# i4Ds/whisper-finetune

Measured on AMD Instinct MI355X. Metric: audio-seconds/sec training throughput, whisper-large-v3 bf16, higher is better.
Workload: dtype bf16; 1 GPU; whisper-large-v3 full fine-tune, AdamW, bf16 MFMA / fp32 master weights, 96 synthetic 30 s clips per GPU per step, decoder S=128, log-mel + SpecAugment on GPU, label smoothing 0.1, clip 1.0, local accumulation 1 (global window = 1); timed loop = model_utils.train_step; global_batch=96, seq_len=128, parallelism=dp1

## Files before the change

### include/wft.h

```cpp
#ifndef WFT_H
#define WFT_H

#include <stdint.h>

#ifdef __cplusplus
extern "C" {
#endif

typedef enum {
  WFT_OK = 0,
  WFT_ERR_ARG = -1,
  WFT_ERR_LAUNCH = -2,
  WFT_ERR_UNSUPPORTED = -3
} wft_status;

typedef uint16_t wft_bf16;

const char* wft_last_error(void);
const char* wft_version(void);

int wft_cast_f32_bf16(const float* src, wft_bf16* dst, int64_t n, void* stream);
int wft_cast_bf16_f32(const wft_bf16* src, float* dst, int64_t n, void* stream);
int wft_cast_pad_transpose_f32_bf16(const float* src, int64_t rows, int64_t cols,
                                    wft_bf16* dst, wft_bf16* dst_t,
// ... 75 lines not shown
} wft_gemm_args;
int wft_gemm_nt_bf16(const wft_gemm_args* args, void* stream);
int wft_gemm_nt_variant(const wft_gemm_args* args);
int wft_gemm_tn_segments_ok(const wft_gemm_args* args);
int64_t wft_gemm_nt_colsum_workspace_bytes(const wft_gemm_args* args);
int64_t wft_gemm_nt_splitk_workspace_bytes(const wft_gemm_args* args);
int64_t wft_gemm_nt_aux8_bytes(const wft_gemm_args* args);
int wft_gemm_nt_stream_bf16(const wft_gemm_args* args, void* stream);
int wft_gemm_nt_stream_ok(const wft_gemm_args* args);
int64_t wft_gemm_nt_stream_workspace_bytes(const wft_gemm_args* args);
int wft_gemm_nt_stream_q8(const wft_gemm_args* args, const float* b_scale, void* stream);
int wft_gemm_nt_stream_q8_ok(const wft_gemm_args* args);
int64_t wft_gemm_nt_stream_q8_workspace_bytes(const wft_gemm_args* args);
int wft_gemm_tn_bf16(const wft_gemm_args* args, void* stream);
int wft_gemm_tn_variant(const wft_gemm_args* args);
int wft_gemm_nt_rank_pair_bf16(const wft_gemm_args* args0, const wft_gemm_args* args1, void* stream);
int wft_gemm_tn_rank_pair_bf16(const wft_gemm_args* args0, const wft_gemm_args* args1, void* stream);
int64_t wft_gemm_tn_workspace_bytes(const wft_gemm_args* args);

typedef struct {
  const wft_bf16* q; int64_t ldq; int64_t q_bs;
  const wft_bf16* k; int64_t ldk; int64_t k_bs;
  const wft_bf16* v; int64_t ldv; int64_t v_bs;
  wft_bf16* o; int64_t ldo; int64_t o_bs;
  float* lse;
  int B; int H; int Tq; int Tk; int causal; float scale;
  const wft_bf16* d_o; int64_t lddo; int64_t do_bs;
  float* delta;
  wft_bf16* dq; int64_t lddq; int64_t dq_bs;
  wft_bf16* dk; int64_t lddk; int64_t dk_bs;
// ... 177 lines not shown
```

### whisper-finetune_amd/csrc/gemm.hip

```cpp
#include "gemm_common.h"
#include <stdlib.h>

struct TnReduceP {
  const float* ws; float* C; long ldc; int P, Q, nsplit, accumulate, Pz; const float* col_scale; int scale_rows, blk_n, blk_r, Pv;
};
__device__ __forceinline__ void tn_splitk_reduce_body(const float* ws, float* C, long ldc, int P, int Q, int nsplit,
                                                      int accumulate, int Pz, const float* col_scale, int scale_rows,
                                                      int blk_n, int blk_r, int Pv, long bid, long nblk) {
  const long nq4 = Q >> 2;
  const long total = (long)(Pz > P ? Pz : P) * nq4;
  for (long i = bid * 256 + threadIdx.x; i < total; i += nblk * 256) {
    const long pp = i / nq4, q4 = (i - pp * nq4) * 4;
    float* cp = C + pp * ldc + q4;
    if (col_scale && blk_n == 0 && pp >= Pv) continue;
    if (pp >= P) {
      if (!accumulate && blk_n == 0) *(f32x4*)cp = f32x4{0.f, 0.f, 0.f, 0.f};
      continue;
    }
    int pr = 0;
    float* ob = nullptr;
    if (blk_n > 0) {
      const int blk = (int)(q4 / blk_n);
      pr = (int)pp - blk * blk_r;
      if (pr < 0 || pr >= blk_r) continue;
      ob = C + (long)blk * blk_n * blk_r + (q4 - (long)blk * blk_n) * blk_r + pr;
    }
    const bool plain = !col_scale && !ob;
    f32x4 s = (plain && accumulate) ? *(const f32x4*)cp : f32x4{0.f, 0.f, 0.f, 0.f};
    for (int k = 0; k < nsplit; ++k) s += *(const f32x4*)(ws + ((long)k * P + pp) * Q + q4);
    if (plain) {
      *(f32x4*)cp = s;
      continue;
    }
    if (col_scale && pp < Pv) s *= *(const f32x4*)(col_scale + (scale_rows > 0 ? pp / scale_rows : 0) * Q + q4);
    if (ob) {
#pragma unroll
      for (int e = 0; e < 4; ++e) ob[(long)e * blk_r] = accumulate ? ob[(long)e * blk_r] + s[e] : s[e];
    } else {
      if (accumulate) s += *(const f32x4*)cp;
      *(f32x4*)cp = s;
    }
  }
}

__global__ __launch_bounds__(256) void tn_splitk_reduce_kernel(const float* ws, float* C, long ldc, int P, int Q, int nsplit,
                                                                int accumulate, int Pz, const float* col_scale, int scale_rows,
                                                                int blk_n, int blk_r, int Pv) {
  tn_splitk_reduce_body(ws, C, ldc, P, Q, nsplit, accumulate, Pz, col_scale, scale_rows, blk_n, blk_r, Pv, (long)blockIdx.x, (long)gridDim.x);
}
struct TnSegs { float* ptr[4]; int end[4]; };
__global__ __launch_bounds__(256) void tn_splitk_reduce_seg_kernel(const float* ws, TnSegs sg, int P, int Q, int nsplit, int accumulate) {
  const long nq4 = Q >> 2;
  const long total = (long)P * nq4;
  for (long i = (long)blockIdx.x * 256 + threadIdx.x; i < total; i += (long)gridDim.x * 256) {
    const long pp = i / nq4, q4 = (i - pp * nq4) * 4;
    int sgi = 0, start = 0;
    while (sgi < 3 && pp >= sg.end[sgi]) start = sg.end[sgi++];
    float* cp = sg.ptr[sgi] + (pp - start) * Q + q4;
    f32x4 s = accumulate ? *(const f32x4*)cp : f32x4{0.f, 0.f, 0.f, 0.f};
    for (int k = 0; k < nsplit; ++k) s += *(const f32x4*)(ws + ((long)k * P + pp) * Q + q4);
    *(f32x4*)cp = s;
  }
}
__global__ __launch_bounds__(256) void tn_splitk_reduce_pair_kernel(TnReduceP r0, TnReduceP r1, int g0) {
  const bool second = (int)blockIdx.x >= g0;
  const TnReduceP& r = second ? r1 : r0;
  tn_splitk_reduce_body(r.ws, r.C, r.ldc, r.P, r.Q, r.nsplit, r.accumulate, r.Pz, r.col_scale, r.scale_rows, r.blk_n, r.blk_r, r.Pv,
                        (long)blockIdx.x - (second ? g0 : 0), (long)(second ? (int)gridDim.x - g0 : g0));
}

static const int g_diag = [] { const char* e = wft_dev_getenv("WFT_GEMM_DIAG"); return e ? atoi(e) : 0; }();
static const int g_nt256_band = [] { const char* e = wft_dev_getenv("WFT_NT256_BAND"); return (e && atoi(e) > 0) ? atoi(e) : 5; }();

static void fill_params(const wft_gemm_args* a, GemmP& p) {
  p.A = a->A; p.lda = a->lda; p.sA = a->strideA;
  p.B = a->B; p.ldb = a->ldb; p.sB = a->strideB;
  p.C = a->C; p.ldc = a->ldc; p.sC = a->strideC;
  p.bias = a->bias;
  p.res = a->residual; p.ldr = a->ldr; p.sR = a->strideR;
  p.aux = a->aux; p.ldaux = a->ldaux; p.sAux = a->strideAux;
  p.alpha = a->alpha;
  p.beta = a->beta == 0.f ? 1.f : a->beta;
  p.M = (int)a->M; p.N = (int)a->N; p.K = (int)a->K; p.batch = a->batch;
  p.accumulate = a->accumulate;
  p.period = a->valid_rows_period; p.valid = a->valid_rows;
  p.res_first = a->residual_first;
  p.diag = g_diag;
  p.band = g_nt256_band;
  p.ws = nullptr;
  p.cs_part = nullptr;
  p.nsplit = 1;
}

static bool ws_granted(const wft_gemm_args* a, int64_t bytes) {
  return a->workspace && a->workspace_bytes >= bytes && (((uintptr_t)a->workspace) & 15) == 0;
}

static int gemm_check_common(const wft_gemm_args* a, const char* who) {
  WFT_CHECK_ARG_AS(who, a->lda % 8 == 0 && a->ldb % 8 == 0 && a->ldc % 4 == 0, "ld alignment");
  WFT_CHECK_ARG_AS(who, ((uintptr_t)a->A & 15) == 0 && ((uintptr_t)a->B & 15) == 0 && ((uintptr_t)a->C & 15) == 0,
                   "base pointers must be 16-byte aligned");
  WFT_CHECK_ARG_AS(who, !(a->accumulate && !a->c_is_f32), "accumulate needs an f32 C");
  return WFT_OK;
}

static const int g_force_128 = [] { const char* e = wft_dev_getenv("WFT_GEMM_FORCE_128"); return (e && e[0] == '1') ? 1 : 0; }();
// ... 108 lines not shown
}

static bool tn_uses_256(const wft_gemm_args* a) {
  const long nsteps = ((a->K + 63) / 64) * a->batch;
  const long t256 = (a->M / 256) * (a->N / 256);
  return !g_force_128 && a->c_is_f32 && a->M % 256 == 0 && a->N % 256 == 0 && nsteps >= g_tn256_min_steps &&
         (nsteps >= 256 || t256 >= g_tn256_min_out_tiles || (t256 >= g_tn256_min_out_tiles / 2 && nsteps >= 128));
}
static bool tn_needs_reduce(const wft_gemm_args* a) { return a->tn_col_scale != nullptr || a->tn_block_n > 0; }
static const int g_tn_variant = [] { const char* e = wft_dev_getenv("WFT_TN_VARIANT"); return (e && e[0] == 'p') ? 1 : 0; }();

struct TnPlan {
  TnKind kind = TN_128_2BUF;
  long tiles = 0;
  int nsplit = 1, per = 0;
  int pb = 0;
  int64_t ws_rows = 0;
  int64_t part_bytes = 0;
  int64_t ws_bytes = 0;
  bool use_ws = false;
};
static TnPlan tn_plan(const wft_gemm_args* a) {
  TnPlan pl;
  if (!a) return pl;
  const bool seg = a->tn_seg_count > 0;
  const auto part = [&](int nsplit) { return (int64_t)nsplit * pl.ws_rows * a->N * 4; };
  if (tn_uses_256(a)) {
    pl.tiles = (a->M / 256) * (a->N / 256);
    pl.ws_rows = a->M;
    const int ns256 = wft_tn256_nsplit(a);
    int ns4 = 0, per4 = 0;
    const bool elig4 = wft_tn4w_eligible(a);
    if (elig4) wft_tn4w_plan(a, &ns4, &per4);
    const int nsq = ns4 > ns256 ? ns4 : ns256;
    pl.ws_bytes = (nsq > 1 || seg || tn_needs_reduce(a)) ? part(nsq) : 0;
    if (elig4 && g_tn_variant != 1 && a->variant == 0) {
      const bool use4 = (ns4 > 1 || seg) && ws_granted(a, part(ns4));
      if (ns4 == 1 || use4) {
        pl.kind = TN_4W; pl.nsplit = ns4; pl.per = per4; pl.use_ws = use4; pl.part_bytes = part(ns4);
        return pl;
      }
    }
    pl.kind = TN_256; pl.nsplit = ns256; pl.part_bytes = part(ns256);
    pl.use_ws = (ns256 > 1 || seg) && ws_granted(a, pl.part_bytes);
    return pl;
  }
  pl.tiles = (a->M / 128) * (a->N / 128);
  const bool ring = wft_tn128_ring(a, g_diag);
  pl.nsplit = wft_tn128_nsplit(a, ring);
  pl.pb = wft_tn128_pb(a);
  pl.ws_rows = pl.pb ? 16 * pl.pb : a->M;
  pl.part_bytes = part(pl.nsplit);
  const bool want_ws = pl.nsplit > 1 || tn_needs_reduce(a);
  pl.ws_bytes = (want_ws || seg) ? pl.part_bytes : 0;
  pl.use_ws = want_ws && ws_granted(a, pl.part_bytes);
  if (pl.pb > 0 && (pl.nsplit == 1 || pl.use_ws)) pl.kind = TN_RANK;
  else if (!a->c_is_f32) pl.kind = TN_128_BF16C;
  else if (pl.pb > 0) pl.kind = TN_128_PB;
  else pl.kind = ring ? TN_128_RING : TN_128_2BUF;
  return pl;
}

extern "C" int wft_gemm_tn_segments_ok(const wft_gemm_args* a) {
  const TnKind k = tn_plan(a).kind;
  if ((k != TN_4W && k != TN_256) || a->tn_seg_count < 1 || a->tn_seg_count > 4 || tn_needs_reduce(a) || a->p_valid != 0 || a->batch != 1) return 0;
  int prev = 0;
  for (int i = 0; i < a->tn_seg_count; ++i) {
    if (a->tn_seg_end[i] <= prev || !a->tn_seg_ptr[i] || (((uintptr_t)a->tn_seg_ptr[i]) & 15) != 0) return 0;
    prev = a->tn_seg_end[i];
  }
  return prev == a->M ? 1 : 0;
}
extern "C" int64_t wft_gemm_tn_workspace_bytes(const wft_gemm_args* a) { return tn_plan(a).ws_bytes; }
extern "C" int wft_gemm_tn_variant(const wft_gemm_args* a) {
  const TnKind k = tn_plan(a).kind;
  return k == TN_4W ? 4 : k == TN_256 ? 256 : 128;
}

static int tn_check(const wft_gemm_args* a, const TnPlan& pl, const char* who) {
  WFT_CHECK_ARG_AS(who, a && a->A && a->B && a->C, "null pointer");
  WFT_CHECK_ARG_AS(who, a->M >= 128 && a->N >= 128 && a->K >= 1 && a->batch >= 1, "bad shape");
  WFT_CHECK_ARG_AS(who, a->M % 128 == 0 && a->N % 128 == 0, "P and Q must be multiples of 128");
  const int rc = gemm_check_common(a, who);
  if (rc != WFT_OK) return rc;
  WFT_CHECK_ARG_AS(who, a->M < (1ll << 31) && a->N < (1ll << 31) && a->K < (1ll << 31), "dims exceed int32");
  if (tn_needs_reduce(a)) {
    WFT_CHECK_ARG_AS(who, pl.pb > 0, "tn_col_scale / tn_block_n need a rank-r operand (P = 128, 0 < p_valid <= 64)");
    WFT_CHECK_ARG_AS(who, ws_granted(a, pl.ws_bytes), "tn_col_scale / tn_block_n need the workspace of wft_gemm_tn_workspace_bytes");
    WFT_CHECK_ARG_AS(who, a->tn_scale_rows >= 0 && (((uintptr_t)a->tn_col_scale) & 15) == 0, "tn_col_scale: 16-byte aligned f32 [S][Q]");
    if (a->tn_block_n > 0)
      WFT_CHECK_ARG_AS(who, a->tn_block_n % 4 == 0 && a->N % a->tn_block_n == 0 && a->tn_block_r >= 1 &&
                       (a->N / a->tn_block_n) * (int64_t)a->tn_block_r <= 16 * pl.pb, "tn_block_n / tn_block_r do not tile the product");
  }
// ... 6 lines not shown
static TnSegs tn_segs_of(const wft_gemm_args* a) {
  TnSegs sg;
  for (int i = 0; i < 4; ++i) {
    const int j = i < a->tn_seg_count ? i : a->tn_seg_count - 1;
    sg.ptr[i] = a->tn_seg_ptr[j];
    sg.end[i] = i < a->tn_seg_count ? a->tn_seg_end[i] : 0x7fffffff;
  }
  return sg;
}
static unsigned tn_reduce_grid(const wft_gemm_args* a) {
  const long g = (a->M * (a->N / 4) + 255) / 256;
  return (unsigned)(g > 2048 ? 2048 : g);
}
static TnReduceP tn_reduce_params(const wft_gemm_args* a, const TnPlan& pl) {
  return TnReduceP{(const float*)a->workspace, (float*)a->C, (long)a->ldc, (int)pl.ws_rows, (int)a->N, pl.nsplit, a->accumulate, (int)a->M,
                   a->tn_col_scale, a->tn_scale_rows, a->tn_block_n, a->tn_block_r, pl.pb > 0 ? a->p_valid : (int)a->M};
}
static void launch_tn_reduce(const wft_gemm_args* a, const TnPlan& pl, hipStream_t s) {
  const dim3 grid(tn_reduce_grid(a)), block(256);
  if (a->tn_seg_count > 0) {
    hipLaunchKernelGGL(tn_splitk_reduce_seg_kernel, grid, block, 0, s, (const float*)a->workspace, tn_segs_of(a), (int)a->M, (int)a->N,
                       pl.nsplit, a->accumulate);
    return;
  }
  const TnReduceP r = tn_reduce_params(a, pl);
  hipLaunchKernelGGL(tn_splitk_reduce_kernel, grid, block, 0, s, r.ws, r.C, r.ldc, r.P, r.Q, r.nsplit, r.accumulate, r.Pz, r.col_scale,
                     r.scale_rows, r.blk_n, r.blk_r, r.Pv);
}

extern "C" int wft_gemm_tn_bf16(const wft_gemm_args* a, void* stream) {
  const TnPlan pl = tn_plan(a);
  int rc = tn_check(a, pl, __func__);
  if (rc != WFT_OK) return rc;
  GemmP p;
  fill_params(a, p);
  hipStream_t s = (hipStream_t)stream;
  if (pl.use_ws) p.ws = (float*)a->workspace;
  else if (pl.nsplit > 1 && !a->accumulate)
    (void)hipMemset2DAsync(a->C, (size_t)a->ldc * 4, 0, (size_t)a->N * 4, (size_t)a->M, s);
  const unsigned grid1d = (unsigned)(pl.tiles * pl.nsplit);
  switch (pl.kind) {
    case TN_4W:
      p.nsplit = pl.nsplit;
      p.band = pl.per;
      rc = wft_tn4w_launch(p, grid1d, stream);
      break;
    case TN_256:
      p.nsplit = pl.nsplit;
      rc = wft_tn256_launch(p, grid1d, s);
      break;
    case TN_RANK:
      p.nsplit = pl.nsplit;
      rc = wft_tn_rank_launch(pl.pb, p, p, (int)grid1d, 0, s);
      break;
    default: rc = wft_tn128_launch(p, pl.kind, pl.pb, dim3((unsigned)pl.tiles, (unsigned)pl.nsplit), s); break;
  }
  if (rc != WFT_OK) return rc;
  if (pl.use_ws) launch_tn_reduce(a, pl, s);
  WFT_CHECK_LAUNCH();
// ... 24 lines not shown
  bool paired = pl[0].pb == pl[1].pb;
  for (int i = 0; i < 2 && paired; ++i)
    paired = pl[i].kind == TN_RANK && ws_granted(as[i], pl[i].part_bytes) && tn_check(as[i], pl[i], __func__) == WFT_OK;
  if (!paired) {
    const int rc = wft_gemm_tn_bf16(a0, stream);
    return rc != WFT_OK ? rc : wft_gemm_tn_bf16(a1, stream);
  }
  hipStream_t s = (hipStream_t)stream;
  GemmP p[2];
  TnReduceP r[2];
  int nb[2], gr[2];
  for (int i = 0; i < 2; ++i) {
    fill_params(as[i], p[i]);
    p[i].ws = (float*)as[i]->workspace;
    p[i].nsplit = pl[i].nsplit;
    nb[i] = (int)(pl[i].tiles * pl[i].nsplit);
    gr[i] = (int)tn_reduce_grid(as[i]);
    r[i] = tn_reduce_params(as[i], pl[i]);
  }
  const int rc = wft_tn_rank_launch(pl[0].pb, p[0], p[1], nb[0], nb[1], s);
  if (rc != WFT_OK) return rc;
  hipLaunchKernelGGL(tn_splitk_reduce_pair_kernel, dim3((unsigned)(gr[0] + gr[1])), dim3(256), 0, s, r[0], r[1], gr[0]);
  WFT_CHECK_LAUNCH();
  return WFT_OK;
}
```

### whisper-finetune_amd/csrc/gemm_common.h

```cpp
#pragma once
#include "common.h"
#include <type_traits>

struct GemmP {
  const unsigned short* A; long lda; long sA;
  const unsigned short* B; long ldb; long sB;
  void* C; long ldc; long sC;
  const float* bias;
  const unsigned short* res; long ldr; long sR;
  unsigned short* aux; long ldaux; long sAux;
  float alpha, beta;
  int M, N, K, batch;
  int accumulate;
  int period, valid;
  int res_first;
  float* ws;
  float* cs_part;
  int nsplit;
  int band;
  int diag;
};

__device__ __forceinline__ void band_coords(int sid, int tiles_r, int tiles_c, int& tr, int& tc, int W = 5) {
  const int band = sid / (tiles_r * W);
  const int c0 = band * W;
  const int w = (tiles_c - c0) < W ? (tiles_c - c0) : W;
  const int r = sid - band * tiles_r * W;
  tr = r / w;
  tc = c0 + r - tr * w;
}

__device__ __forceinline__ int xcd_remap(int bid, int ntile) {
  const int q = ntile >> 3, r = ntile & 7, xcd = bid & 7;
  return (xcd < r ? xcd * (q + 1) : r * (q + 1) + (xcd - r) * q) + (bid >> 3);
}

template <int IMM>
__device__ __forceinline__ bf16x8 lds_b128_asm(unsigned lds_byte_addr) {
  bf16x8 r;
  asm volatile("ds_read_b128 %0, %1 offset:%2" : "=v"(r) : "v"(lds_byte_addr), "n"(IMM));
  return r;
}
template <int IMM>
__device__ __forceinline__ s16x4 tn_tr_asm(unsigned lds_byte_addr) {
// ... 53 lines not shown
    case WFT_EPI_NONE: return either(EpiC<WFT_EPI_NONE>{});
    case WFT_EPI_GELU: return either(EpiC<WFT_EPI_GELU>{});
    case WFT_EPI_DGELU: return either(EpiC<WFT_EPI_DGELU>{});
    case WFT_EPI_GELU_GRAD: return f(EpiC<WFT_EPI_GELU_GRAD>{}, std::false_type{});
    case WFT_EPI_MUL_AUX: return f(EpiC<WFT_EPI_MUL_AUX>{}, std::false_type{});
    default: wft_set_error("wft_gemm_nt_bf16: unknown epilogue %d", a->epilogue); return WFT_ERR_ARG;
  }
}

enum NtKind { NT_4W, NT_256, NT_RANK, NT_128_SPLITK, NT_128_RING, NT_128_2BUF };
enum TnKind { TN_4W, TN_256, TN_RANK, TN_128_PB, TN_128_RING, TN_128_2BUF, TN_128_BF16C };
bool wft_nt4w_eligible(const wft_gemm_args* a);
int wft_nt4w_launch(const wft_gemm_args* a, const GemmP& p, unsigned grid, void* stream);
bool wft_tn4w_eligible(const wft_gemm_args* a);
void wft_tn4w_plan(const wft_gemm_args* a, int* nsplit_out, int* per_out);
int wft_tn4w_launch(const GemmP& p, unsigned grid, void* stream);
int wft_nt256_launch(const wft_gemm_args* a, const GemmP& p, unsigned grid, hipStream_t s);
void wft_nt_colsum_reduce_launch(const wft_gemm_args* a, hipStream_t s);
int wft_tn256_nsplit(const wft_gemm_args* a);
int wft_tn256_launch(const GemmP& p, unsigned grid, hipStream_t s);
bool wft_nt128_ring(const wft_gemm_args* a, int diag);
int wft_nt128_splitk_plan(const wft_gemm_args* a, int diag, int* per_out);
int wft_nt128_launch(const wft_gemm_args* a, const GemmP& p, NtKind kind, int nsplit, int per, dim3 grid, hipStream_t s);
bool wft_tn128_ring(const wft_gemm_args* a, int diag);
int wft_tn128_nsplit(const wft_gemm_args* a, bool ring);
int wft_tn128_pb(const wft_gemm_args* a);
int wft_tn128_launch(const GemmP& p, TnKind kind, int pb, dim3 grid, hipStream_t s);
int wft_nt_rank_pb(const wft_gemm_args* a);
int wft_nt_rank_launch(int pb, const GemmP& p0, const GemmP& p1, int n0, int n1, hipStream_t s);
int wft_tn_rank_launch(int pb, const GemmP& p0, const GemmP& p1, int n0, int n1, hipStream_t s);
// ... 1 lines not shown
```

### whisper-finetune_amd/csrc/gemm_tn4w.hip

```cpp
#include "gemm_common.h"
#include <stdlib.h>
#include <type_traits>

#define TN4W_BLK 1056
#define TN4W_OP (32 * TN4W_BLK)
#define TN4W_BUF (2 * TN4W_OP)
#define TN4W_LDS (2 * TN4W_BUF)

#define TN4W_STR2(x) #x
#define TN4W_STR(x) TN4W_STR2(x)

#ifndef TN4W_SPP
#define TN4W_SPP 12
#endif
#ifndef TN4W_SPQ
#define TN4W_SPQ 12
#endif
#define TN4W_ASM_MACROS ".set TN4W_SPP, " TN4W_STR(TN4W_SPP) "\n.set TN4W_SPQ, " TN4W_STR(TN4W_SPQ) "\n" R"ASM(
.macro TN4W_MFMA s, z
  .if \z
    v_mfma_f32_16x16x32_bf16 a[4*((\s)%%64):4*((\s)%%64)+3], v[128+64*((\s)/64)+4*((\s)%%8):128+64*((\s)/64)+4*((\s)%%8)+3], v[160+64*((\s)/64)+4*(((\s)%%64)/8):160+64*((\s)/64)+4*(((\s)%%64)/8)+3], 0
  .else
    v_mfma_f32_16x16x32_bf16 a[4*((\s)%%64):4*((\s)%%64)+3], v[128+64*((\s)/64)+4*((\s)%%8):128+64*((\s)/64)+4*((\s)%%8)+3], v[160+64*((\s)/64)+4*(((\s)%%64)/8):160+64*((\s)/64)+4*(((\s)%%64)/8)+3], a[4*((\s)%%64):4*((\s)%%64)+3]
  .endif
// ... 240 lines not shown
__device__ __forceinline__ unsigned tn4w_sgpr(unsigned x) { return __builtin_amdgcn_readfirstlane(x); }
__device__ __forceinline__ unsigned long long tn4w_sgpr64(unsigned long long x) {
  const unsigned lo = __builtin_amdgcn_readfirstlane((unsigned)x), hi = __builtin_amdgcn_readfirstlane((unsigned)(x >> 32));
  return ((unsigned long long)hi << 32) | lo;
}

__global__ __launch_bounds__(256) void gemm_tn4w_kernel(GemmP p) {
  extern __shared__ __attribute__((aligned(16))) char dsmem[];
  const int tid = threadIdx.x, lane = tid & 63;
  const int wave = __builtin_amdgcn_readfirstlane(tid >> 6);
  const int wp = wave >> 1, wq = wave & 1;
  const int P = p.M, Q = p.N, R = p.K;
  const int tiles_q = Q >> 8, tiles_p = P >> 8;
  const int ntile = tiles_p * tiles_q;
  const int nsplit = p.nsplit;
  const int wsid = xcd_remap(blockIdx.x, ntile * nsplit);
  const int split = wsid / ntile, sid = wsid - split * ntile;
  int tp, tq;
  band_coords(sid, tiles_p, tiles_q, tp, tq);
  const int p0 = tp << 8, q0 = tq << 8;
  const int per = p.band;
  const int kb = split * per;
  const int nk_all = (((R + 63) >> 6) + 1) & ~1;
  const int nk = (kb + per <= nk_all) ? per : nk_all - kb;
  const unsigned lds0 = lds_addr_of(dsmem);
  const unsigned lda2 = tn4w_sgpr((unsigned)p.lda * 2u), ldb2 = tn4w_sgpr((unsigned)p.ldb * 2u);

  const int g = lane >> 4, li = lane & 15;
  const unsigned rd0 = lds0 + (unsigned)((li >> 2) + 4 * (g & 1) + 16 * (g >> 1)) * TN4W_BLK + 8u * (li & 3);
  const unsigned rdP0 = rd0 + wp * 256, rdQ0 = rd0 + TN4W_OP + wq * 256;
  const int h = lane >> 5, cp = lane & 31;
  const int rw = 32 * h + 16 * (wave >> 1) + 4 * (wave & 1);
  const unsigned voP = (unsigned)(rw * (int)p.lda + cp * 8) * 2u, voQ = (unsigned)(rw * (int)p.ldb + cp * 8) * 2u;
  const unsigned long long baseP = tn4w_sgpr64((unsigned long long)(p.A + (long)kb * 64 * p.lda + p0));
  const unsigned long long baseQ = tn4w_sgpr64((unsigned long long)(p.B + (long)kb * 64 * p.ldb + q0));
  const long rem = (long)R - (long)kb * 64;
  const unsigned nrP = tn4w_sgpr((unsigned)(rem * p.lda * 2)), nrQ = tn4w_sgpr((unsigned)(rem * p.ldb * 2));
  tn4w_kloop(rdP0, rdQ0, voP, voQ, baseP, baseQ, nrP, nrQ, lda2, ldb2, tn4w_sgpr(lds0 + wave * 8 * TN4W_BLK),
             tn4w_sgpr((unsigned)(nk - 4) >> 1));

  float* const dst = p.ws ? p.ws + ((long)split * P + p0) * Q + q0 : (float*)p.C + (long)p0 * p.ldc + q0;
  const long ldd = p.ws ? (long)Q : p.ldc;
  const bool acc_c = !p.ws && p.accumulate;
  tn4w_for<0, 8>([&](auto fpc) {
    constexpr int fp = decltype(fpc)::value;
    float* const row = dst + (long)(wp * 128 + 16 * fp + li) * ldd + wq * 128 + 4 * g;
    tn4w_for<0, 8>([&](auto fqc) {
      constexpr int fq = decltype(fqc)::value, i0 = (fp * 8 + fq) * 4;
      f32x4 o = {tn4w_acc<i0>(), tn4w_acc<i0 + 1>(), tn4w_acc<i0 + 2>(), tn4w_acc<i0 + 3>()};
      o *= p.alpha;
      if (acc_c) o += *(const f32x4*)(row + 16 * fq);
      *(f32x4*)(row + 16 * fq) = o;
    });
  });
}

bool wft_tn4w_eligible(const wft_gemm_args* a) {
  return a->c_is_f32 && a->batch == 1 && a->M % 256 == 0 && a->N % 256 == 0 && a->K >= 1024 && a->p_valid == 0 && !a->tn_col_scale &&
         a->tn_block_n == 0 && a->lda >= a->M && a->ldb >= a->N && (a->K + 64) * a->lda * 2 < (1ll << 32) &&
         (a->K + 64) * a->ldb * 2 < (1ll << 32);
}
void wft_tn4w_plan(const wft_gemm_args* a, int* nsplit_out, int* per_out) {
  const long t256 = (a->M / 256) * (a->N / 256);
  const long nk = ((((a->K + 63) / 64) + 1) / 2) * 2;
  const int ncu = wft_num_cus();
  int nsplit = 1;
  double best = 0.0;
  for (int sp = 1; sp <= 16; ++sp) {
    if (sp > 1 && nk / sp < 24) break;
    const double waves = (double)(t256 * sp) / (double)ncu;
    const double eff = waves / (double)((long)(waves + 0.999999));
    if (eff > best + 0.02) { best = eff; nsplit = sp; }
  }
  long per = (nk + nsplit - 1) / nsplit;
  per = (per + 1) & ~1l;
  if (per < 4) per = 4;
  long ns = (nk + per - 1) / per;
  while (ns > 1 && nk - (ns - 1) * per < 4) {
    per += 2;
    ns = (nk + per - 1) / per;
  }
  *per_out = (int)per;
  *nsplit_out = (int)ns;
}
int wft_tn4w_launch(const GemmP& p, unsigned grid, void* stream) {
  return wft_launch_lds<gemm_tn4w_kernel>(dim3(grid), dim3(256), TN4W_LDS, (hipStream_t)stream, p);
}
```

### whisper-finetune_amd/whisper_finetune/engine/kernels.py

```python
from __future__ import annotations

import ctypes as C
import math
from typing import Optional

import torch

from . import lib as L

BF16 = torch.bfloat16
F32 = torch.float32

PROFILE_NT = None


def _p(t: Optional[torch.Tensor]):
    return C.c_void_p(0 if t is None else t.data_ptr())


def _chk(t: torch.Tensor, dtype, name: str):
    if t.dtype != dtype:
        raise TypeError(f"{name}: expected {dtype}, got {t.dtype}")
    if not t.is_cuda:
        raise L.WftError(f"{name}: libwft kernels need CUDA/HIP tensors (got {t.device}); there is no CPU path")
# ... 207 lines not shown
            "wft_layernorm_bwd",
        )
    if want_colsum:
        return dx, dgamma, dbeta, dxs
    return dx, dgamma, dbeta


VARIANT = {"nt": 0, "tn": 0, "fwd": 0, "dq": 0, "dkdv": 0}
LAUNCH_OVERRIDE = [None]
LAUNCH_PERSISTENT, LAUNCH_PER_TILE = 0, 1


def set_variant(which: str, v: int) -> int:
    old = VARIANT[which]
    if v >= 0:
        VARIANT[which] = 1 if v else 0
    return old


def _launch(launch: int) -> int:
    o = LAUNCH_OVERRIDE[0]
    return int(launch) if o is None else int(o)


def _attn_variant_bits() -> int:
    return VARIANT["fwd"] | (VARIANT["dq"] << 1) | (VARIANT["dkdv"] << 2)


def gemm_nt(a, b, *, M=None, N=None, K=None, lda=None, ldb=None, out=None, out_f32=False, accumulate=False,
            bias=None, residual=None, aux=None, epilogue=L.EPI_NONE, alpha=1.0, batch=1,
            strideA=0, strideB=0, strideC=0, strideR=0, strideAux=0, ldc=None,
# ... 993 lines not shown
```

### whisper-finetune_amd/whisper_finetune/engine/lib.py

```python
from __future__ import annotations

import ctypes as C
import os
from pathlib import Path

_PKG_ROOT = Path(__file__).resolve().parents[2]
LIB_PATH = Path(os.environ.get("WFT_LIB", _PKG_ROOT / "libwft.so"))

c_i64 = C.c_int64
c_vp = C.c_void_p


class GemmArgs(C.Structure):

    _fields_ = [
        ("A", c_vp), ("lda", c_i64), ("strideA", c_i64),
        ("B", c_vp), ("ldb", c_i64), ("strideB", c_i64),
        ("C", c_vp), ("ldc", c_i64), ("strideC", c_i64), ("c_is_f32", C.c_int), ("accumulate", C.c_int),
        ("bias", c_vp),
        ("residual", c_vp), ("ldr", c_i64), ("strideR", c_i64),
        ("aux", c_vp), ("ldaux", c_i64), ("strideAux", c_i64),
        ("epilogue", C.c_int), ("alpha", C.c_float),
        ("M", c_i64), ("N", c_i64), ("K", c_i64), ("batch", C.c_int),
        ("valid_rows_period", C.c_int), ("valid_rows", C.c_int),
# ... 140 lines not shown
                                C.c_int, c_vp, c_vp],
    "wft_gemm_nt_bf16": [C.POINTER(GemmArgs), c_vp],
    "wft_gemm_nt_variant": [C.POINTER(GemmArgs)],
    "wft_gemm_tn_segments_ok": [C.POINTER(GemmArgs)],
    "wft_gemm_nt_colsum_workspace_bytes": [C.POINTER(GemmArgs)],
    "wft_gemm_nt_splitk_workspace_bytes": [C.POINTER(GemmArgs)],
    "wft_gemm_nt_aux8_bytes": [C.POINTER(GemmArgs)],
    "wft_gemm_nt_stream_bf16": [C.POINTER(GemmArgs), c_vp],
    "wft_gemm_nt_stream_ok": [C.POINTER(GemmArgs)],
    "wft_gemm_nt_stream_workspace_bytes": [C.POINTER(GemmArgs)],
    "wft_gemm_nt_stream_q8": [C.POINTER(GemmArgs), c_vp, c_vp],
    "wft_gemm_nt_stream_q8_ok": [C.POINTER(GemmArgs)],
    "wft_gemm_nt_stream_q8_workspace_bytes": [C.POINTER(GemmArgs)],
    "wft_gemm_tn_bf16": [C.POINTER(GemmArgs), c_vp],
    "wft_gemm_tn_variant": [C.POINTER(GemmArgs)],
    "wft_gemm_nt_rank_pair_bf16": [C.POINTER(GemmArgs), C.POINTER(GemmArgs), c_vp],
    "wft_gemm_tn_rank_pair_bf16": [C.POINTER(GemmArgs), C.POINTER(GemmArgs), c_vp],
    "wft_gemm_tn_workspace_bytes": [C.POINTER(GemmArgs)],
    "wft_attn_fwd_bf16": [C.POINTER(AttnArgs), c_vp],
    "wft_attn_bwd_bf16": [C.POINTER(AttnArgs), c_vp],
    "wft_attn_bwd_colsum_workspace_bytes": [C.POINTER(AttnArgs)],
    "wft_attn_variant": [C.POINTER(AttnArgs), C.c_int],
    "wft_attn_decode_bf16": [C.POINTER(AttnDecodeArgs), c_vp],
    "wft_attn_decode_workspace_bytes": [C.POINTER(AttnDecodeArgs)],
    "wft_decode_embed": [c_vp, c_i64, c_vp, c_vp, c_vp, c_vp, C.c_int, C.c_int, C.c_int, c_i64, c_vp],
    "wft_decode_pick": [C.POINTER(DecodePickArgs), c_vp],
    "wft_attn_decode_beam_bf16": [C.POINTER(AttnDecodeBeamArgs), c_vp],
    "wft_attn_decode_beam_workspace_bytes": [C.POINTER(AttnDecodeBeamArgs)],
    "wft_decode_topk": [C.POINTER(DecodeTopkArgs), c_vp],
    "wft_decode_pick_ts": [C.POINTER(DecodePickArgs), C.POINTER(TsRules), c_vp],
# ... 105 lines not shown
```

Measured before the change: 3620 audio-s/s.

## Add stream-K style balanced split-K scheduling for TN 4-wave weight-gradient GEMM

Adds a balanced work decomposition for the TN 4-wave GEMM. When there are fewer 256x256 tiles than CUs and K is long, each CU gets an equal share of K-steps, and workgroups may walk across tile boundaries into several partial-sum slots. The split-K reduce kernels now work out a per-tile part count so they sum only the slots that were written. This aims to remove wave-quantization tail imbalance in weight-gradient GEMMs. In exchange it adds extra workspace slots, a per-segment fixed cost, and more complex indexing in the kernel and the reduction.

```diff
diff --git a/include/wft.h b/include/wft.h
--- a/include/wft.h
+++ b/include/wft.h
@@ -113,6 +113,10 @@
 int64_t wft_gemm_nt_stream_q8_workspace_bytes(const wft_gemm_args* args);
 int wft_gemm_tn_bf16(const wft_gemm_args* args, void* stream);
 int wft_gemm_tn_variant(const wft_gemm_args* args);
+int wft_gemm_tn_plan(const wft_gemm_args* args, int* out);
+int wft_tn_balanced_segments(int T, int nk, int G, int c, int wg, int* out, int max_segs);
+int wft_tn_balanced_parts(int T, int nk, int G, int c, int tile);
+int wft_tn_balanced_seg_cost(void);
 int wft_gemm_nt_rank_pair_bf16(const wft_gemm_args* args0, const wft_gemm_args* args1, void* stream);
 int wft_gemm_tn_rank_pair_bf16(const wft_gemm_args* args0, const wft_gemm_args* args1, void* stream);
 int64_t wft_gemm_tn_workspace_bytes(const wft_gemm_args* args);
diff --git a/whisper-finetune_amd/csrc/gemm.hip b/whisper-finetune_amd/csrc/gemm.hip
--- a/whisper-finetune_amd/csrc/gemm.hip
+++ b/whisper-finetune_amd/csrc/gemm.hip
@@ -1,12 +1,19 @@
 #include "gemm_common.h"
 #include <stdlib.h>
+#include <algorithm>
 
 struct TnReduceP {
   const float* ws; float* C; long ldc; int P, Q, nsplit, accumulate, Pz; const float* col_scale; int scale_rows, blk_n, blk_r, Pv;
+  int bal_G, bal_nk;
 };
+__device__ __forceinline__ int tn_balanced_parts_at(const TnbPlan& bp, int P, int Q, long pp, long q4) {
+  return tnb_tile_parts(bp, band_index((int)(pp >> 8), (int)(q4 >> 8), P >> 8, Q >> 8));
+}
 __device__ __forceinline__ void tn_splitk_reduce_body(const float* ws, float* C, long ldc, int P, int Q, int nsplit,
                                                       int accumulate, int Pz, const float* col_scale, int scale_rows,
-                                                      int blk_n, int blk_r, int Pv, long bid, long nblk) {
+                                                      int blk_n, int blk_r, int Pv, int bal_G, int bal_nk, long bid, long nblk) {
+  TnbPlan bp;
+  const bool bal = bal_G > 0 && tnb_make((P >> 8) * (Q >> 8), bal_nk, bal_G, TNB_SEG_COST, bp);
   const long nq4 = Q >> 2;
   const long total = (long)(Pz > P ? Pz : P) * nq4;
   for (long i = bid * 256 + threadIdx.x; i < total; i += nblk * 256) {
@@ -27,7 +34,8 @@
     }
     const bool plain = !col_scale && !ob;
     f32x4 s = (plain && accumulate) ? *(const f32x4*)cp : f32x4{0.f, 0.f, 0.f, 0.f};
-    for (int k = 0; k < nsplit; ++k) s += *(const f32x4*)(ws + ((long)k * P + pp) * Q + q4);
+    const int ns = bal ? tn_balanced_parts_at(bp, P, Q, pp, q4) : nsplit;
+    for (int k = 0; k < ns; ++k) s += *(const f32x4*)(ws + ((long)k * P + pp) * Q + q4);
     if (plain) {
       *(f32x4*)cp = s;
       continue;
@@ -45,11 +53,15 @@
 
 __global__ __launch_bounds__(256) void tn_splitk_reduce_kernel(const float* ws, float* C, long ldc, int P, int Q, int nsplit,
                                                                 int accumulate, int Pz, const float* col_scale, int scale_rows,
-                                                                int blk_n, int blk_r, int Pv) {
-  tn_splitk_reduce_body(ws, C, ldc, P, Q, nsplit, accumulate, Pz, col_scale, scale_rows, blk_n, blk_r, Pv, (long)blockIdx.x, (long)gridDim.x);
+                                                                int blk_n, int blk_r, int Pv, int bal_G, int bal_nk) {
+  tn_splitk_reduce_body(ws, C, ldc, P, Q, nsplit, accumulate, Pz, col_scale, scale_rows, blk_n, blk_r, Pv, bal_G, bal_nk, (long)blockIdx.x,
+                        (long)gridDim.x);
 }
 struct TnSegs { float* ptr[4]; int end[4]; };
-__global__ __launch_bounds__(256) void tn_splitk_reduce_seg_kernel(const float* ws, TnSegs sg, int P, int Q, int nsplit, int accumulate) {
+__global__ __launch_bounds__(256) void tn_splitk_reduce_seg_kernel(const float* ws, TnSegs sg, int P, int Q, int nsplit, int accumulate,
+                                                                    int bal_G, int bal_nk) {
+  TnbPlan bp;
+  const bool bal = bal_G > 0 && tnb_make((P >> 8) * (Q >> 8), bal_nk, bal_G, TNB_SEG_COST, bp);
   const long nq4 = Q >> 2;
   const long total = (long)P * nq4;
   for (long i = (long)blockIdx.x * 256 + threadIdx.x; i < total; i += (long)gridDim.x * 256) {
@@ -58,7 +70,8 @@
     while (sgi < 3 && pp >= sg.end[sgi]) start = sg.end[sgi++];
     float* cp = sg.ptr[sgi] + (pp - start) * Q + q4;
     f32x4 s = accumulate ? *(const f32x4*)cp : f32x4{0.f, 0.f, 0.f, 0.f};
-    for (int k = 0; k < nsplit; ++k) s += *(const f32x4*)(ws + ((long)k * P + pp) * Q + q4);
+    const int ns = bal ? tn_balanced_parts_at(bp, P, Q, pp, q4) : nsplit;
+    for (int k = 0; k < ns; ++k) s += *(const f32x4*)(ws + ((long)k * P + pp) * Q + q4);
     *(f32x4*)cp = s;
   }
 }
@@ -66,7 +79,7 @@
   const bool second = (int)blockIdx.x >= g0;
   const TnReduceP& r = second ? r1 : r0;
   tn_splitk_reduce_body(r.ws, r.C, r.ldc, r.P, r.Q, r.nsplit, r.accumulate, r.Pz, r.col_scale, r.scale_rows, r.blk_n, r.blk_r, r.Pv,
-                        (long)blockIdx.x - (second ? g0 : 0), (long)(second ? (int)gridDim.x - g0 : g0));
+                        r.bal_G, r.bal_nk, (long)blockIdx.x - (second ? g0 : 0), (long)(second ? (int)gridDim.x - g0 : g0));
 }
 
 static const int g_diag = [] { const char* e = wft_dev_getenv("WFT_GEMM_DIAG"); return e ? atoi(e) : 0; }();
@@ -90,6 +103,7 @@
   p.ws = nullptr;
   p.cs_part = nullptr;
   p.nsplit = 1;
+  p.balanced = 0;
 }
 
 static bool ws_granted(const wft_gemm_args* a, int64_t bytes) {
@@ -228,6 +242,8 @@
   TnKind kind = TN_128_2BUF;
   long tiles = 0;
   int nsplit = 1, per = 0;
+  bool balanced = false;
+  unsigned grid = 0;
   int pb = 0;
   int64_t ws_rows = 0;
   int64_t part_bytes = 0;
@@ -243,19 +259,27 @@
     pl.tiles = (a->M / 256) * (a->N / 256);
     pl.ws_rows = a->M;
     const int ns256 = wft_tn256_nsplit(a);
-    int ns4 = 0, per4 = 0;
+    int ns4 = 0, per4 = 0, nsb = 0, perb = 0, gridb = 0;
     const bool elig4 = wft_tn4w_eligible(a);
     if (elig4) wft_tn4w_plan(a, &ns4, &per4);
-    const int nsq = ns4 > ns256 ? ns4 : ns256;
+    const bool bal = elig4 && wft_tn4w_balanced(a, ns4, per4, &nsb, &perb, &gridb);
+    const int nsq = std::max(std::max(ns4, ns256), nsb);
     pl.ws_bytes = (nsq > 1 || seg || tn_needs_reduce(a)) ? part(nsq) : 0;
-    if (elig4 && g_tn_variant != 1 && a->variant == 0) {
+    if (elig4 && g_tn_variant != 1 && (a->variant == 0 || a->variant == 2)) {
+      if (bal && a->variant == 0 && ws_granted(a, part(nsb))) {
+        pl.kind = TN_4W; pl.balanced = true; pl.nsplit = nsb; pl.per = perb; pl.use_ws = true; pl.part_bytes = part(nsb);
+        pl.grid = (unsigned)gridb;
+        return pl;
+      }
       const bool use4 = (ns4 > 1 || seg) && ws_granted(a, part(ns4));
       if (ns4 == 1 || use4) {
         pl.kind = TN_4W; pl.nsplit = ns4; pl.per = per4; pl.use_ws = use4; pl.part_bytes = part(ns4);
+        pl.grid = (unsigned)(pl.tiles * ns4);
         return pl;
       }
     }
     pl.kind = TN_256; pl.nsplit = ns256; pl.part_bytes = part(ns256);
+    pl.grid = (unsigned)(pl.tiles * ns256);
     pl.use_ws = (ns256 > 1 || seg) && ws_granted(a, pl.part_bytes);
     return pl;
   }
@@ -265,6 +289,7 @@
   pl.pb = wft_tn128_pb(a);
   pl.ws_rows = pl.pb ? 16 * pl.pb : a->M;
   pl.part_bytes = part(pl.nsplit);
+  pl.grid = (unsigned)(pl.tiles * pl.nsplit);
   const bool want_ws = pl.nsplit > 1 || tn_needs_reduce(a);
   pl.ws_bytes = (want_ws || seg) ? pl.part_bytes : 0;
   pl.use_ws = want_ws && ws_granted(a, pl.part_bytes);
@@ -291,6 +316,12 @@
   return k == TN_4W ? 4 : k == TN_256 ? 256 : 128;
 }
 
+extern "C" int wft_gemm_tn_plan(const wft_gemm_args* a, int* out) {
+  const TnPlan pl = tn_plan(a);
+  out[0] = pl.balanced ? 1 : 0; out[1] = (int)pl.grid; out[2] = pl.nsplit; out[3] = pl.kind == TN_4W ? pl.per : 0;
+  return wft_gemm_tn_variant(a);
+}
+
 static int tn_check(const wft_gemm_args* a, const TnPlan& pl, const char* who) {
   WFT_CHECK_ARG_AS(who, a && a->A && a->B && a->C, "null pointer");
   WFT_CHECK_ARG_AS(who, a->M >= 128 && a->N >= 128 && a->K >= 1 && a->batch >= 1, "bad shape");
@@ -327,18 +358,19 @@
 }
 static TnReduceP tn_reduce_params(const wft_gemm_args* a, const TnPlan& pl) {
   return TnReduceP{(const float*)a->workspace, (float*)a->C, (long)a->ldc, (int)pl.ws_rows, (int)a->N, pl.nsplit, a->accumulate, (int)a->M,
-                   a->tn_col_scale, a->tn_scale_rows, a->tn_block_n, a->tn_block_r, pl.pb > 0 ? a->p_valid : (int)a->M};
+                   a->tn_col_scale, a->tn_scale_rows, a->tn_block_n, a->tn_block_r, pl.pb > 0 ? a->p_valid : (int)a->M,
+                   pl.balanced ? (int)pl.grid : 0, (int)((((a->K + 63) / 64 + 1) / 2) * 2)};
 }
 static void launch_tn_reduce(const wft_gemm_args* a, const TnPlan& pl, hipStream_t s) {
   const dim3 grid(tn_reduce_grid(a)), block(256);
+  const TnReduceP r = tn_reduce_params(a, pl);
   if (a->tn_seg_count > 0) {
     hipLaunchKernelGGL(tn_splitk_reduce_seg_kernel, grid, block, 0, s, (const float*)a->workspace, tn_segs_of(a), (int)a->M, (int)a->N,
-                       pl.nsplit, a->accumulate);
+                       pl.nsplit, a->accumulate, r.bal_G, r.bal_nk);
     return;
   }
-  const TnReduceP r = tn_reduce_params(a, pl);
   hipLaunchKernelGGL(tn_splitk_reduce_kernel, grid, block, 0, s, r.ws, r.C, r.ldc, r.P, r.Q, r.nsplit, r.accumulate, r.Pz, r.col_scale,
-                     r.scale_rows, r.blk_n, r.blk_r, r.Pv);
+                     r.scale_rows, r.blk_n, r.blk_r, r.Pv, r.bal_G, r.bal_nk);
 }
 
 extern "C" int wft_gemm_tn_bf16(const wft_gemm_args* a, void* stream) {
@@ -351,11 +383,12 @@
   if (pl.use_ws) p.ws = (float*)a->workspace;
   else if (pl.nsplit > 1 && !a->accumulate)
     (void)hipMemset2DAsync(a->C, (size_t)a->ldc * 4, 0, (size_t)a->N * 4, (size_t)a->M, s);
-  const unsigned grid1d = (unsigned)(pl.tiles * pl.nsplit);
+  const unsigned grid1d = pl.grid;
   switch (pl.kind) {
     case TN_4W:
       p.nsplit = pl.nsplit;
       p.band = pl.per;
+      p.balanced = pl.balanced ? 1 : 0;
       rc = wft_tn4w_launch(p, grid1d, stream);
       break;
     case TN_256:
@@ -410,7 +443,7 @@
     fill_params(as[i], p[i]);
     p[i].ws = (float*)as[i]->workspace;
     p[i].nsplit = pl[i].nsplit;
-    nb[i] = (int)(pl[i].tiles * pl[i].nsplit);
+    nb[i] = (int)pl[i].grid;
     gr[i] = (int)tn_reduce_grid(as[i]);
     r[i] = tn_reduce_params(as[i], pl[i]);
   }
diff --git a/whisper-finetune_amd/csrc/gemm_common.h b/whisper-finetune_amd/csrc/gemm_common.h
--- a/whisper-finetune_amd/csrc/gemm_common.h
+++ b/whisper-finetune_amd/csrc/gemm_common.h
@@ -1,5 +1,6 @@
 #pragma once
 #include "common.h"
+#include "tn_balanced.h"
 #include <type_traits>
 
 struct GemmP {
@@ -19,6 +20,7 @@
   int nsplit;
   int band;
   int diag;
+  int balanced;
 };
 
 __device__ __forceinline__ void band_coords(int sid, int tiles_r, int tiles_c, int& tr, int& tc, int W = 5) {
@@ -28,6 +30,12 @@
   const int r = sid - band * tiles_r * W;
   tr = r / w;
   tc = c0 + r - tr * w;
+}
+
+__device__ __forceinline__ int band_index(int tr, int tc, int tiles_r, int tiles_c, int W = 5) {
+  const int band = tc / W, c0 = band * W;
+  const int w = (tiles_c - c0) < W ? (tiles_c - c0) : W;
+  return band * tiles_r * W + tr * w + (tc - c0);
 }
 
 __device__ __forceinline__ int xcd_remap(int bid, int ntile) {
@@ -111,6 +119,7 @@
 int wft_nt4w_launch(const wft_gemm_args* a, const GemmP& p, unsigned grid, void* stream);
 bool wft_tn4w_eligible(const wft_gemm_args* a);
 void wft_tn4w_plan(const wft_gemm_args* a, int* nsplit_out, int* per_out);
+bool wft_tn4w_balanced(const wft_gemm_args* a, int ns, int per, int* slots_out, int* steps_out, int* grid_out);
 int wft_tn4w_launch(const GemmP& p, unsigned grid, void* stream);
 int wft_nt256_launch(const wft_gemm_args* a, const GemmP& p, unsigned grid, hipStream_t s);
 void wft_nt_colsum_reduce_launch(const wft_gemm_args* a, hipStream_t s);
diff --git a/whisper-finetune_amd/csrc/gemm_tn4w.hip b/whisper-finetune_amd/csrc/gemm_tn4w.hip
--- a/whisper-finetune_amd/csrc/gemm_tn4w.hip
+++ b/whisper-finetune_amd/csrc/gemm_tn4w.hip
@@ -278,15 +278,22 @@
   const int tiles_q = Q >> 8, tiles_p = P >> 8;
   const int ntile = tiles_p * tiles_q;
   const int nsplit = p.nsplit;
-  const int wsid = xcd_remap(blockIdx.x, ntile * nsplit);
-  const int split = wsid / ntile, sid = wsid - split * ntile;
-  int tp, tq;
-  band_coords(sid, tiles_p, tiles_q, tp, tq);
-  const int p0 = tp << 8, q0 = tq << 8;
-  const int per = p.band;
-  const int kb = split * per;
   const int nk_all = (((R + 63) >> 6) + 1) & ~1;
-  const int nk = (kb + per <= nk_all) ? per : nk_all - kb;
+  TnbPlan bp;
+  TnbWalk wk;
+  if (p.balanced) {
+    tnb_make(ntile, nk_all, (int)gridDim.x, TNB_SEG_COST, bp);
+    const int nfull = bp.s * ntile;
+    wk = tnb_walk(bp, (int)blockIdx.x < nfull ? xcd_remap(blockIdx.x, nfull) : (int)blockIdx.x);
+  } else {
+    const int wsid = xcd_remap(blockIdx.x, ntile * nsplit);
+    const int split = wsid / ntile, per = p.band;
+    bp.nk = nk_all;
+    wk.t0 = wk.t1 = wsid - split * ntile;
+    wk.k_first = wk.k_mid = split * per;
+    wk.k_last = (wk.k_first + per <= nk_all) ? wk.k_first + per : nk_all;
+    wk.slot_first = wk.slot_mid = split;
+  }
   const unsigned lds0 = lds_addr_of(dsmem);
   const unsigned lda2 = tn4w_sgpr((unsigned)p.lda * 2u), ldb2 = tn4w_sgpr((unsigned)p.ldb * 2u);
 
@@ -296,27 +303,37 @@
   const int h = lane >> 5, cp = lane & 31;
   const int rw = 32 * h + 16 * (wave >> 1) + 4 * (wave & 1);
   const unsigned voP = (unsigned)(rw * (int)p.lda + cp * 8) * 2u, voQ = (unsigned)(rw * (int)p.ldb + cp * 8) * 2u;
-  const unsigned long long baseP = tn4w_sgpr64((unsigned long long)(p.A + (long)kb * 64 * p.lda + p0));
-  const unsigned long long baseQ = tn4w_sgpr64((unsigned long long)(p.B + (long)kb * 64 * p.ldb + q0));
-  const long rem = (long)R - (long)kb * 64;
-  const unsigned nrP = tn4w_sgpr((unsigned)(rem * p.lda * 2)), nrQ = tn4w_sgpr((unsigned)(rem * p.ldb * 2));
-  tn4w_kloop(rdP0, rdQ0, voP, voQ, baseP, baseQ, nrP, nrQ, lda2, ldb2, tn4w_sgpr(lds0 + wave * 8 * TN4W_BLK),
-             tn4w_sgpr((unsigned)(nk - 4) >> 1));
-
-  float* const dst = p.ws ? p.ws + ((long)split * P + p0) * Q + q0 : (float*)p.C + (long)p0 * p.ldc + q0;
   const long ldd = p.ws ? (long)Q : p.ldc;
   const bool acc_c = !p.ws && p.accumulate;
-  tn4w_for<0, 8>([&](auto fpc) {
-    constexpr int fp = decltype(fpc)::value;
-    float* const row = dst + (long)(wp * 128 + 16 * fp + li) * ldd + wq * 128 + 4 * g;
-    tn4w_for<0, 8>([&](auto fqc) {
-      constexpr int fq = decltype(fqc)::value, i0 = (fp * 8 + fq) * 4;
-      f32x4 o = {tn4w_acc<i0>(), tn4w_acc<i0 + 1>(), tn4w_acc<i0 + 2>(), tn4w_acc<i0 + 3>()};
-      o *= p.alpha;
-      if (acc_c) o += *(const f32x4*)(row + 16 * fq);
-      *(f32x4*)(row + 16 * fq) = o;
+  for (int sid = tn4w_sgpr((unsigned)wk.t0); sid <= wk.t1; ++sid) {
+    const TnbSeg sg = tnb_walk_seg(bp, wk, sid - wk.t0);
+    const int kb = sg.k0, nk = sg.n;
+    int tp, tq;
+    band_coords(sid, tiles_p, tiles_q, tp, tq);
+    const int p0 = tp << 8, q0 = tq << 8;
+    const unsigned long long baseP = tn4w_sgpr64((unsigned long long)(p.A + (long)kb * 64 * p.lda + p0));
+    const unsigned long long baseQ = tn4w_sgpr64((unsigned long long)(p.B + (long)kb * 64 * p.ldb + q0));
+    const long rem = (long)R - (long)kb * 64;
+    const unsigned nrP = tn4w_sgpr((unsigned)(rem * p.lda * 2)), nrQ = tn4w_sgpr((unsigned)(rem * p.ldb * 2));
+    tn4w_kloop(rdP0, rdQ0, voP, voQ, baseP, baseQ, nrP, nrQ, lda2, ldb2, tn4w_sgpr(lds0 + wave * 8 * TN4W_BLK),
+               tn4w_sgpr((unsigned)(nk - 4) >> 1));
+
+    float* const dst = p.ws ? p.ws + ((long)sg.slot * P + p0) * Q + q0 : (float*)p.C + (long)p0 * p.ldc + q0;
+    tn4w_for<0, 8>([&](auto fpc) {
+      constexpr int fp = decltype(fpc)::value;
+      float* const row = dst + (long)(wp * 128 + 16 * fp + li) * ldd + wq * 128 + 4 * g;
+      tn4w_for<0, 8>([&](auto fqc) {
+        constexpr int fq = decltype(fqc)::value, i0 = (fp * 8 + fq) * 4;
+        f32x4 o = {tn4w_acc<i0>(), tn4w_acc<i0 + 1>(), tn4w_acc<i0 + 2>(), tn4w_acc<i0 + 3>()};
+        o *= p.alpha;
+        if (acc_c) o += *(const f32x4*)(row + 16 * fq);
+        *(f32x4*)(row + 16 * fq) = o;
+      });
     });
-  });
+    if (sid == wk.t1) break;
+    asm volatile("s_waitcnt vmcnt(0)" ::: "memory");
+    __syncthreads();
+  }
 }
 
 bool wft_tn4w_eligible(const wft_gemm_args* a) {
@@ -347,6 +364,40 @@
   *per_out = (int)per;
   *nsplit_out = (int)ns;
 }
+#define TNB_MIN_STEPS 256
+bool wft_tn4w_balanced(const wft_gemm_args* a, int ns, int per, int* slots_out, int* steps_out, int* grid_out) {
+  const long t256 = (a->M / 256) * (a->N / 256);
+  const long nk = ((((a->K + 63) / 64) + 1) / 2) * 2;
+  const int ncu = wft_num_cus();
+  TnbPlan bp;
+  if (t256 > ncu || nk < TNB_MIN_STEPS || !tnb_make((int)t256, (int)nk, ncu, TNB_SEG_COST, bp)) return false;
+  if (bp.s + 2 > ns) return false;
+  const long rounds = (t256 * ns + ncu - 1) / ncu;
+  const long t_uniform = rounds * (per + TNB_SEG_COST), t_balanced = bp.L + TNB_SEG_COST;
+  if (t_balanced * 100 >= t_uniform * 96) return false;
+  *slots_out = bp.s + 2;
+  *steps_out = bp.L;
+  *grid_out = ncu;
+  return true;
+}
+extern "C" int wft_tn_balanced_segments(int T, int nk, int G, int c, int wg, int* out, int max_segs) {
+  TnbPlan bp;
+  if (!tnb_make(T, nk, G, c < 0 ? TNB_SEG_COST : c, bp) || wg < 0 || wg >= G) return -1;
+  const TnbWalk w = tnb_walk(bp, wg);
+  int n = 0;
+  for (int t = w.t0; t <= w.t1; ++t, ++n) {
+    if (n >= max_segs) return -1;
+    const TnbSeg sg = tnb_walk_seg(bp, w, t - w.t0);
+    out[4 * n] = sg.tile; out[4 * n + 1] = sg.k0; out[4 * n + 2] = sg.n; out[4 * n + 3] = sg.slot;
+  }
+  return n;
+}
+extern "C" int wft_tn_balanced_parts(int T, int nk, int G, int c, int tile) {
+  TnbPlan bp;
+  if (!tnb_make(T, nk, G, c < 0 ? TNB_SEG_COST : c, bp) || tile < 0 || tile >= T) return -1;
+  return tnb_tile_parts(bp, tile);
+}
+extern "C" int wft_tn_balanced_seg_cost(void) { return TNB_SEG_COST; }
 int wft_tn4w_launch(const GemmP& p, unsigned grid, void* stream) {
   return wft_launch_lds<gemm_tn4w_kernel>(dim3(grid), dim3(256), TN4W_LDS, (hipStream_t)stream, p);
 }
diff --git a/whisper-finetune_amd/csrc/tn_balanced.h b/whisper-finetune_amd/csrc/tn_balanced.h
--- /dev/null
+++ b/whisper-finetune_amd/csrc/tn_balanced.h
@@ -0,0 +1,88 @@
+#pragma once
+
+#if defined(__HIPCC__)
+#define TNB_HD __host__ __device__ __forceinline__
+#else
+#define TNB_HD static inline
+#endif
+
+#ifndef TNB_SEG_COST
+#define TNB_SEG_COST 15
+#endif
+
+struct TnbPlan {
+  int T, nk, G, c;
+  int s, r;
+  int L, rest;
+};
+struct TnbCut { int tile, off; };
+struct TnbSeg { int tile, k0, n, slot; };
+
+TNB_HD bool tnb_make(int T, int nk, int G, int c, TnbPlan& pl) {
+  pl.T = T; pl.nk = nk; pl.G = G; pl.c = c;
+  pl.s = pl.r = pl.L = pl.rest = 0;
+  if (T < 1 || T > G || nk < 4 || (nk & 1) || c < 0) return false;
+  pl.s = G / T;
+  pl.r = G - pl.s * T;
+  if (pl.r == 0) return false;
+  const long long num = (long long)T * (nk + c);
+  pl.L = (int)(((num + G - 1) / G + 1) & ~1ll);
+  pl.rest = nk - pl.s * pl.L;
+  if (pl.L < 4 || pl.rest < 8) return false;
+  if ((long long)pl.r * T * (pl.rest + c) >= (1ll << 31)) return false;
+  return true;
+}
+
+TNB_HD TnbCut tnb_cut(const TnbPlan& pl, int h) {
+  TnbCut cu;
+  if (h <= 0) { cu.tile = 0; cu.off = 0; return cu; }
+  if (h >= pl.r) { cu.tile = pl.T; cu.off = 0; return cu; }
+  const unsigned U = (unsigned)(pl.rest + pl.c);
+  const unsigned v = (unsigned)h * ((unsigned)pl.T * U) / (unsigned)pl.r;
+  const unsigned t = v / U, u = v - t * U;
+  int off = u > (unsigned)pl.c ? (int)(u - (unsigned)pl.c) & ~1 : 0;
+  cu.tile = (int)t;
+  if (off < 4) off = 0;
+  else if (pl.rest - off < 4) { cu.tile += 1; off = 0; }
+  cu.off = off;
+  return cu;
+}
+
+TNB_HD int tnb_tile_parts(const TnbPlan& pl, int tile) {
+  const int h = (tile * pl.r + pl.T - 1) / pl.T;
+  if (h < 1 || h >= pl.r) return pl.s + 1;
+  const TnbCut cu = tnb_cut(pl, h);
+  return pl.s + 1 + ((cu.tile == tile && cu.off > 0) ? 1 : 0);
+}
+
+struct TnbWalk { int t0, t1, k_first, k_last, k_mid, slot_first, slot_mid; };
+TNB_HD TnbWalk tnb_walk(const TnbPlan& pl, int wg) {
+  TnbWalk w;
+  const int nfull = pl.s * pl.T;
+  if (wg < nfull) {
+    const int j = wg / pl.T;
+    w.t0 = w.t1 = wg - j * pl.T;
+    w.k_first = w.k_mid = j * pl.L;
+    w.k_last = (j + 1) * pl.L;
+    w.slot_first = w.slot_mid = j;
+    return w;
+  }
+  const TnbCut a = tnb_cut(pl, wg - nfull), b = tnb_cut(pl, wg - nfull + 1);
+  const int base = pl.s * pl.L;
+  w.t0 = a.tile;
+  w.k_first = base + a.off;
+  w.slot_first = pl.s + (a.off > 0 ? 1 : 0);
+  w.k_mid = base;
+  w.slot_mid = pl.s;
+  if (b.off > 0) { w.t1 = b.tile; w.k_last = base + b.off; }
+  else { w.t1 = b.tile - 1; w.k_last = pl.nk; }
+  return w;
+}
+TNB_HD TnbSeg tnb_walk_seg(const TnbPlan& pl, const TnbWalk& w, int i) {
+  TnbSeg sg;
+  sg.tile = w.t0 + i;
+  sg.k0 = i == 0 ? w.k_first : w.k_mid;
+  sg.n = (sg.tile == w.t1 ? w.k_last : pl.nk) - sg.k0;
+  sg.slot = i == 0 ? w.slot_first : w.slot_mid;
+  return sg;
+}
diff --git a/whisper-finetune_amd/whisper_finetune/engine/kernels.py b/whisper-finetune_amd/whisper_finetune/engine/kernels.py
--- a/whisper-finetune_amd/whisper_finetune/engine/kernels.py
+++ b/whisper-finetune_amd/whisper_finetune/engine/kernels.py
@@ -245,7 +245,7 @@
 def set_variant(which: str, v: int) -> int:
     old = VARIANT[which]
     if v >= 0:
-        VARIANT[which] = 1 if v else 0
+        VARIANT[which] = 2 if (which == "tn" and v == 2) else (1 if v else 0)
     return old
 
 
diff --git a/whisper-finetune_amd/whisper_finetune/engine/lib.py b/whisper-finetune_amd/whisper_finetune/engine/lib.py
--- a/whisper-finetune_amd/whisper_finetune/engine/lib.py
+++ b/whisper-finetune_amd/whisper_finetune/engine/lib.py
@@ -178,6 +178,10 @@
     "wft_gemm_nt_stream_q8_workspace_bytes": [C.POINTER(GemmArgs)],
     "wft_gemm_tn_bf16": [C.POINTER(GemmArgs), c_vp],
     "wft_gemm_tn_variant": [C.POINTER(GemmArgs)],
+    "wft_gemm_tn_plan": [C.POINTER(GemmArgs), C.POINTER(C.c_int)],
+    "wft_tn_balanced_segments": [C.c_int, C.c_int, C.c_int, C.c_int, C.c_int, C.POINTER(C.c_int), C.c_int],
+    "wft_tn_balanced_parts": [C.c_int, C.c_int, C.c_int, C.c_int, C.c_int],
+    "wft_tn_balanced_seg_cost": [],
     "wft_gemm_nt_rank_pair_bf16": [C.POINTER(GemmArgs), C.POINTER(GemmArgs), c_vp],
     "wft_gemm_tn_rank_pair_bf16": [C.POINTER(GemmArgs), C.POINTER(GemmArgs), c_vp],
     "wft_gemm_tn_workspace_bytes": [C.POINTER(GemmArgs)],
```

After: 3625 audio-s/s (median of 4 runs). Within noise of the previous version (+0.2%).
